# santurini/vsrlab

Measured on AMD Instinct MI355X. Metric: LR frames/sec fwd+bwd, BasicVSR 4x 540p 7-frame clip, 1->8 MI355X, higher is better.
Workload: dtype bf16; 1 GPU; BasicVSR(mid=64,res_blocks=30,x4) fwd+Charbonnier+bwd+clip+Adam, 540x960->2160x3840, 7-frame clip, 2 clips per GPU (BASELINE configs[1]); clips_per_gpu=2, frames=7, res_blocks=30, parallelism=single GPU, arena=full, train_flow=False, trunk_chains=True

## Files before the change

### vsrlab_amd/csrc/common.h

```cpp
#pragma once
#include <hip/hip_runtime.h>
#include <stdint.h>

#define VSR_OK 0
#define VSR_ERR_BADARG (-1)
#define VSR_ERR_UNSUPPORTED (-2)
#define VSR_ERR_HIP (-3)
#define VSR_ERR_WORKSPACE (-4)

#define VSR_F32 0
#define VSR_BF16 1

typedef __bf16 bf16_t;
typedef __attribute__((ext_vector_type(8))) __bf16 bf16x8_t;
typedef __attribute__((ext_vector_type(4))) __bf16 bf16x4_t;
typedef __attribute__((ext_vector_type(4))) short s16x4_t;
typedef __attribute__((ext_vector_type(16))) float f32x16_t;
typedef __attribute__((ext_vector_type(4))) float f32x4_t;

#define VSR_MAX_SRC 4
#define VSR_MAX_Z 4

enum { ACT_NONE = 0, ACT_RELU = 1, ACT_LEAKY = 2 };
enum { MASK_NONE = 0, MASK_RELU = 1, MASK_LEAKY = 2, MASK_RELU_BITS = 3, MASK_LEAKY_BITS = 4 };
enum { EPI_NHWC = 0, EPI_PLANAR = 1 };

struct ConvArgs {
    const void* src[VSR_MAX_SRC];
    long long src_nstride[VSR_MAX_SRC];
    int src_oy[VSR_MAX_SRC], src_ox[VSR_MAX_SRC];
    int in_step, Hs, Ws;
    int N, H, W;
    const void* wpack;
    long long w_zstride;
    const float* bias;
    int bias_zstride;
    int nz;
    void* dst[VSR_MAX_Z];
    long long dst_nstride;
    int out_step, Hd, Wd;
    int out_oy[VSR_MAX_Z], out_ox[VSR_MAX_Z];
    int CD;
    int cout_real;
    int act;
    const void* res[VSR_MAX_Z];
    const void* aux[VSR_MAX_Z];
    int mask_mode;
    const float* pres;
    const float* base_lr;
    long long base_nstride;
    int base_h, base_w, base_scale;
    void* sign_out[VSR_MAX_Z];
    const void* sign_bits[VSR_MAX_Z];
    float leaky_slope;
    int planar_c;
    int unshuffle;
    long long unshuffle_plane;
};
static inline __host__ __device__ float vsr_slope(float s) { return s != 0.f ? s : 0.1f; }

#define VSR_WG_MAXSEG 8
struct WgradArgs {
    const void* x[VSR_WG_MAXSEG];
    const void* dy[VSR_WG_MAXSEG];
    long long x_nstride, dy_nstride;
    int nseg;
    int N, H, W;
    int x_step, x_oy, x_ox, Hx, Wx;
    int dy_step, dy_oy, dy_ox, Hy, Wy;
    float* slab;
    int tap_begin;
    int x_ctotal, x_coff;
    int dy_ctotal, dy_coff;
    int dy_planar_c;
    int slab_stride;
    int ntiles_x, ntiles_y;
    int pair_ksplit, pair_nsl, pair_ncob, pair_views;
};

static inline __host__ __device__ int cdiv(int a, int b) { return (a + b - 1) / b; }

static inline __host__ __device__ int pm_ws(int W) { return (W + 31) >> 5; }
static inline __host__ __device__ long long pm_image_elems(int H, int W, int C) { return (long long)H * pm_ws(W) * 32 * C; }
static inline __host__ __device__ long long pm_off(int y, int x, int chunk, int W, int C) {
    const int seg = x >> 5;
    return (((long long)y * pm_ws(W) + seg) * (C >> 3) + chunk) * 256 + (x & 31) * 8;
}

static inline __host__ __device__ int pm_acc_chan(int mb, int row) { return 8 * (4 * (mb >> 1) + (row >> 2)) + 4 * (mb & 1) + (row & 3); }
#define PM_LANE_PIXEL(l15) (((l15) >= 4 && (l15) < 12) ? 2 * ((l15) - 4) : ((l15) < 4 ? 2 * (l15) + 1 : 2 * ((l15) - 8) + 1))

struct TileWalk { int first, end, stride; };
static inline __device__ TileWalk xcd_tile_walk(int total, int block, int nblocks) {
    TileWalk w;
    if (nblocks >= 8 && (nblocks & 7) == 0) {
        const int xcd = block & 7, j = block >> 3;
        const int lo = (int)((long long)xcd * total / 8), hi = (int)((long long)(xcd + 1) * total / 8);
        w.first = lo + j; w.end = hi; w.stride = nblocks >> 3;
    } else {
        w.first = block; w.end = total; w.stride = nblocks;
    }
    return w;
}

#define VSR_MAX_DEVICES 32
struct VsrDevOnce { bool done[VSR_MAX_DEVICES] = {}; };
static inline int vsr_set_max_dynamic_lds(VsrDevOnce& once, const void* kernel, int bytes) {
    int dev = 0;
    if (hipGetDevice(&dev) != hipSuccess) return VSR_ERR_HIP;
    if (dev < 0 || dev >= VSR_MAX_DEVICES) return VSR_ERR_UNSUPPORTED;
    if (!__atomic_load_n(&once.done[dev], __ATOMIC_ACQUIRE)) {
        if (hipFuncSetAttribute(kernel, hipFuncAttributeMaxDynamicSharedMemorySize, bytes) != hipSuccess) return VSR_ERR_HIP;
        __atomic_store_n(&once.done[dev], true, __ATOMIC_RELEASE);
    }
    return VSR_OK;
}

static inline int vsr_num_cus() {
    static int cus[VSR_MAX_DEVICES] = {};
    int dev = 0;
    if (hipGetDevice(&dev) != hipSuccess || dev < 0 || dev >= VSR_MAX_DEVICES) return 256;
    int v = __atomic_load_n(&cus[dev], __ATOMIC_RELAXED);
    if (v == 0) {
        hipDeviceProp_t prop;
        v = (hipGetDeviceProperties(&prop, dev) == hipSuccess && prop.multiProcessorCount > 0) ? prop.multiProcessorCount : 256;
        __atomic_store_n(&cus[dev], v, __ATOMIC_RELAXED);
    }
    return v;
}

#include <cstdlib>
struct VsrEnvSwitches {
    bool generic_conv, generic_wgrad, single_stream;
    int wide2_max_wg;
};
static inline const VsrEnvSwitches& vsr_env() {
    static const VsrEnvSwitches s = [] {
        auto on = [](const char* n) { const char* e = getenv(n); return e && e[0] == '1'; };
        VsrEnvSwitches v;
        v.generic_conv = on("VSRLAB_AMD_GENERIC_CONV");
        v.generic_wgrad = on("VSRLAB_AMD_GENERIC_WGRAD");
        v.single_stream = on("VSRLAB_AMD_SINGLE_STREAM");
        const char* e = getenv("VSRLAB_AMD_WIDE2_MAX_WG");
        v.wide2_max_wg = e ? atoi(e) : 0;
        return v;
    }();
    return s;
}

#define HIP_CHECK_RET(expr)                                   \
    do {                                                      \
        hipError_t _e = (expr);                               \
        if (_e != hipSuccess) return VSR_ERR_HIP;             \
    } while (0)
```

### vsrlab_amd/csrc/kernels.h

```cpp
#pragma once
#include "common.h"

int vsr_launch_conv(int dtype, int ks, int nsrc, int ca, int cb, int last_planar, int cout_t, int epi,
                    const ConvArgs& a, hipStream_t st);
int vsr_launch_sign_bits_c64(const void* x_pm, void* bits, int N, int H, int W, hipStream_t st);

enum { CHAIN_RELU = 0,
       CHAIN_SKIP = 1,
       CHAIN_MASK = 2 };
#define VSR_CHAIN_MAX_LAYERS 64
struct ChainLayer { unsigned src, dst, res, sbits, sout, w, bias; int variant; };
struct ChainArgs {
    char* base;
    unsigned* sync;
    int N, H, W, nlayers;
    ChainLayer layer[VSR_CHAIN_MAX_LAYERS];
};
size_t vsr_chain_sync_bytes(int nlayers, int N, int H, int W);
int vsr_launch_conv3x3_chain(const ChainArgs& a, int num_cus, hipStream_t st);
void vsr_wgrad_slab_dims(int ks, int cx, int cout, int* coutp, int* cxp, int* stride);
int vsr_launch_wgrad(int dtype, int ks, int cx, int x_planar, int cout, int dy_planar, const WgradArgs& a, int nwg,
                     int* nslabs, hipStream_t st);
int vsr_launch_wgrad_reduce(const float* slab, int nwg, int ks, int cx, int cout, int cout_real, int cin_real, float* gw,
                            int I_total, int i_off, int o_mul, int o_add, float* gb, int accumulate, hipStream_t st);
int vsr_launch_warp_fwd(int dtype, const void* in, const float* flow, void* out, int N, int H, int W, int C,
                        long long flow_nstride, hipStream_t st, int border = 0);
int vsr_launch_warp_bwd(int dtype, const void* dout, const float* flow, float* dacc, int N, int H, int W, int C,
                        long long flow_nstride, hipStream_t st, int border = 0);
int vsr_launch_warp_bwd_gather(int dtype, const void* dout, const float* flow, const void* dtop, long long* S, int* far_count, void* out,
                               int N, int H, int W, int C, long long flow_nstride, hipStream_t st);
int vsr_launch_add_cast(int dtype, const void* a, const float* s, void* out, int N, int H, int W, int C, hipStream_t st);
int vsr_launch_planar_to_pm(int dtype, const float* in, void* out, int N, int Cin, int H, int W, int C, hipStream_t st);
int vsr_launch_pm_to_planar(int dtype, const void* in, float* out, int N, int Cout, int H, int W, int C, hipStream_t st);
int vsr_launch_resize_norm(const float* in, float* out, const float* mean, const float* std, int F, int h, int w, int hu,
                           int wu, hipStream_t st);
int vsr_launch_avgpool2(const float* in, float* out, long long planes, int h, int w, hipStream_t st);
int vsr_launch_spynet_prepare(int dtype, const float* frames, const float* flow_prev, float* flow_up, void* x16, int n,
                              int t, int P, int pair_mode, int h, int w, int level0, hipStream_t st);
int vsr_launch_flow_out(const float* in, float* out, int P, int hu, int wu, int h, int w, hipStream_t st);
int vsr_launch_warp_bwd_flow(int dtype, const void* in, const void* dout, const float* flow, float* dflow, int N, int H, int W,
                             int C, long long flow_nstride, hipStream_t st, int border = 0);
int vsr_launch_spynet_dres(int dtype, const float* dflow, const float* res, void* out, int P, int h, int w, hipStream_t st);
int vsr_launch_spynet_prepare_bwd(int dtype, const void* dx16, const float* dflow_l, const float* frames, const float* flow_up,
                                  float* dflow_prev, float* dframes, int n, int t, int P, int pair_mode, int h, int w, hipStream_t st);
int vsr_launch_avgpool2_bwd_add(const float* dcoarse, float* dfine, long long planes, int h, int w, hipStream_t st);
int vsr_launch_resize_norm_bwd(const float* dnorm, float* dframes, const float* std, int F, int h, int w, int hu, int wu, hipStream_t st);
int vsr_launch_bilinear4_bwd(const float* dsr, float* dlr, long long planes, int h, int w, hipStream_t st, int scale = 4);
int vsr_launch_flow_out_bwd(const float* dout, float* din, int P, int hu, int wu, int h, int w, hipStream_t st);
int vsr_launch_add_f32(const float* a, const float* b, float* out, long long n, hipStream_t st);
int vsr_launch_c64_to_planar(const ConvArgs& a, hipStream_t st);
int vsr_launch_last2_wgrad(const void* x, const float* dy, long long dy_nstride, float* slab, int slab_stride, int N, int H, int W,
                           int* nslabs, hipStream_t st, int pc = 3);
int vsr_launch_last2_dgrad(const float* dsr, long long dsr_nstride, const float* w, const void* aux, void* dst, int N, int H, int W,
                           int mask_mode, hipStream_t st, const void* sign_bits = nullptr, float slope = 0.f);
struct VsrPackDesc {
    const float* w; void* dst;
    int total, blk0;
    short KK, RP, CPd, r_real, c_real, I_total, i_off, o_mul, o_add;
    unsigned char mode, dtype;
};
#define VSR_PACK_BATCH 80
int vsr_launch_pack_multi(const VsrPackDesc* descs, int n, hipStream_t st);
int vsr_launch_pack_weights(int dtype, const float* w, void* dst, int KK, int RP, int CPd, int r_real, int c_real,
                            int I_total, int i_off, int o_mul, int o_add, int mode, hipStream_t st);
int vsr_charbonnier_scratch_floats_impl();
int vsr_launch_charbonnier_grad(const float* sr, const float* hr, float* dsr, float* loss_acc, float* scratch, long long n, float eps,
                                hipStream_t st);

struct VsrWideConv {
    const void* x; int xC, Hx, Wx, in_step, nsl;
    int N, H, W;
    const void* wpack; const float* bias;
    void* y; int yC, Hy, Wy, out_step, ncob;
    int act; float slope;
    void* y_act; const void* res; void* y_pre; const void* aux;
    const void* wpack2;
};
// ... 15 lines not shown
```

### vsrlab_amd/csrc/recipes.h

```cpp
#pragma once
#include <vector>
#include "host.h"

inline constexpr int NSPY = 5;
inline constexpr int SPY_CI[NSPY] = {8, 32, 64, 32, 16};
inline constexpr int SPY_CO[NSPY] = {32, 64, 32, 16, 2};
inline constexpr int SPY_CIP[NSPY] = {16, 32, 64, 32, 16};
inline constexpr int SPY_COP[NSPY] = {32, 64, 32, 32, 32};
inline constexpr int SPY_CD[NSPY] = {32, 64, 32, 16, 0};
inline constexpr int SPY_DK[NSPY] = {32, 64, 32, 16, 16};
inline constexpr int SPY_DROWS[NSPY] = {32, 32, 64, 32, 32};

struct Ctx {
    char* ws;
    hipStream_t st;
    int dtype;
    int C, CO;
    size_t es;
    float* slab;
    mutable std::vector<VsrPackDesc>* batch = nullptr;
    Ctx(char* ws_, hipStream_t st_, int dtype_, int C_ = 64, float* slab_ = nullptr)
        : ws(ws_), st(st_), dtype(dtype_), C(C_), CO(C_ < 32 ? 32 : C_), es(esize(dtype_)), slab(slab_) {}
    void* at(size_t off) const { return ws + off; }
    const float* fat(size_t off) const { return reinterpret_cast<const float*>(ws + off); }
// ... 10 lines not shown
        if (unshuffle) set_unshuffle(a, N, H, W);
        const int rc = vsr_launch_conv(dtype, ks, 1, C, C, 0, CO, EPI_NHWC, a, st);
        if (rc == VSR_OK && sign_out && dtype == VSR_BF16 && vsr_env().generic_conv) return vsr_launch_sign_bits_c64(y, sign_out, N, H, W, st);
        return rc;
    }
    int conv_planar3(const void* x, const void* wpack, const float* bias, float* y, long long y_nstride, const float* pres, int N, int H, int W) const {
        ConvArgs a = conv_args(N, H, W, C);
        a.src[0] = x; a.wpack = wpack; a.bias = bias; a.cout_real = 3; a.dst[0] = y; a.dst_nstride = y_nstride; a.pres = pres;
        return vsr_launch_conv(dtype, 3, 1, C, C, 0, 32, EPI_PLANAR, a, st);
    }

    int pack_ps(const float* w, void* dst, int mode) const {
        for (int z = 0; z < 4; ++z) CK(pack(w, (char*)dst + (size_t)z * 9 * CO * C * es, 9, CO, C, C, C, C, 0, 4, z, mode));
        return VSR_OK;
    }
    int pack_ps_bias(const float* b, float* dst) const {
        for (int z = 0; z < 4; ++z) CK(pack_bias(b, dst + z * C, C, 4, z));
        return VSR_OK;
    }
    int conv_ps(const void* x, const void* wpack, const float* bias4, void* y, int N, int H, int W, int act = ACT_NONE, float slope = 0.f) const {
        ConvArgs a = conv_args(N, H, W, C);
        a.src[0] = x; a.wpack = wpack; a.w_zstride = 9 * CO * C; a.bias = bias4; a.bias_zstride = C; a.nz = 4; a.act = act; a.leaky_slope = slope;
        a.out_step = 2; a.Hd = 2 * H; a.Wd = 2 * W; a.dst_nstride = pm_image_elems(2 * H, 2 * W, C);
        for (int z = 0; z < 4; ++z) { a.dst[z] = y; a.out_oy[z] = z >> 1; a.out_ox[z] = z & 1; }
        return vsr_launch_conv(dtype, 3, 1, C, C, 0, CO, EPI_NHWC, a, st);
    }
    int conv_ps_dgrad(const void* dy, const void* wpackd, void* dx, const void* aux, int mask, int N, int H, int W, const void* sign_bits = nullptr,
                      bool dy_planes = false, bool dx_planes = false) const {
        if (dtype == VSR_BF16 && C == 64) {
            for (int z = 0; z < 4; ++z) {
                ConvArgs a = conv_args(N, H, W, C);
                if (dy_planes) {
                    a.src[0] = (const char*)dy + (size_t)z * plane_elems(N, 2 * H, 2 * W) * es;
                } else {
                    a.in_step = 2; a.Hs = 2 * H; a.Ws = 2 * W;
                    a.src[0] = dy; a.src_oy[0] = z >> 1; a.src_ox[0] = z & 1; a.src_nstride[0] = pm_image_elems(2 * H, 2 * W, C);
                }
                a.wpack = (const char*)wpackd + (size_t)z * 9 * C * C * es; a.dst[0] = dx;
                a.res[0] = z > 0 ? dx : nullptr;
                if (dx_planes) set_unshuffle(a, N, H, W);
                if (z == 3) { a.aux[0] = aux; a.mask_mode = mask; a.sign_bits[0] = aux ? sign_bits : nullptr; }
                int rc = vsr_launch_conv(dtype, 3, 1, 64, 64, 0, 64, EPI_NHWC, a, st);
                if (rc != VSR_OK) return rc;
            }
            return VSR_OK;
        }
        ConvArgs a = conv_args(N, H, W, C);
        a.nz = 1; a.in_step = 2; a.Hs = 2 * H; a.Ws = 2 * W;
        for (int s = 0; s < 4; ++s) { a.src[s] = dy; a.src_oy[s] = s >> 1; a.src_ox[s] = s & 1; a.src_nstride[s] = pm_image_elems(2 * H, 2 * W, C); }
        a.wpack = wpackd; a.dst[0] = dx; a.aux[0] = aux; a.mask_mode = mask;
        return vsr_launch_conv(dtype, 3, 4, C, C, 0, CO, EPI_NHWC, a, st);
    }
    int ps_wgrads(const void* const* x, const void* const* dy, int nseg, bool dy_planes, int N, int H, int W, float* gw, float* gb, int accumulate) const {
        for (int z = 0; z < 4; ++z) {
            WgradArgs a = wg_base(N, H, W, C, C);
            a.nseg = nseg;
            for (int i = 0; i < nseg; ++i) {
                a.x[i] = x[i];
                a.dy[i] = dy_planes ? (const char*)dy[i] + (size_t)z * plane_elems(N, 2 * H, 2 * W) * es : dy[i];
            }
            if (!dy_planes) { a.dy_step = 2; a.dy_oy = z >> 1; a.dy_ox = z & 1; a.Hy = 2 * H; a.Wy = 2 * W; a.dy_nstride = pm_image_elems(2 * H, 2 * W, C); }
            CK(wgrad(a, {3, C, false, C, false}, {C, C, gw, C, 0, 4, z, gb, accumulate}));
        }
        return VSR_OK;
    }

    int pack_stem(const float* w, void* dst, bool cat) const {
        const int I_total = cat ? C + 3 : 3;
        if (cat) CK(pack(w, dst, 9, CO, C, C, C, I_total, 3, 1, 0, 0));
        return pack(w, (char*)dst + (cat ? (size_t)9 * CO * C * es : 0), 9, CO, 16, C, 3, I_total, 0, 1, 0, 0);
    }
    int pack_stem_dgrad(const float* w, void* dst) const { return pack(w, dst, 9, CO, C, C, C, C + 3, 3, 1, 0, 1); }
    int pack_stem_dlr(const float* w, void* dst, bool cat) const { return pack(w, dst, 9, 32, C, 3, C, cat ? C + 3 : 3, 0, 1, 0, 1); }
    int stem(bool cat, const void* feat, const float* lr, long long lr_nstride, const void* wpack, const float* bias, void* y, int act, float slope,
             int N, int H, int W) const {
        ConvArgs a = conv_args(N, H, W, C);
        a.wpack = wpack; a.bias = bias; a.dst[0] = y; a.act = act; a.leaky_slope = slope;
        a.src[cat ? 1 : 0] = lr; a.src_nstride[cat ? 1 : 0] = lr_nstride;
        if (!cat) return vsr_launch_conv(dtype, 3, 1, 16, 16, 1, CO, EPI_NHWC, a, st);
        a.src[0] = feat;
        return vsr_launch_conv(dtype, 3, 2, C, 16, 1, CO, EPI_NHWC, a, st);
    }
    int stem_wgrads(bool cat, WgradArgs& a_lr, WgradArgs& a_feat, float* gw, float* gb, int accumulate) const {
        const int I_total = cat ? C + 3 : 3;
        CK(wgrad(a_lr, {3, 16, true, C, false}, {C, 3, gw, I_total, 0, 1, 0, gb, accumulate}));
        if (cat && a_feat.nseg) CK(wgrad_cc(3, a_feat, gw, I_total, 3, nullptr, accumulate));
        return VSR_OK;
    }

    int pack_spy(int j, const float* w, void* dst, int mode) const {
        if (mode == 0) return pack(w, dst, 49, SPY_COP[j], SPY_CIP[j], SPY_CO[j], SPY_CI[j], SPY_CI[j], 0, 1, 0, 0);
        return pack(w, dst, 49, SPY_DROWS[j], SPY_DK[j], SPY_CI[j], SPY_CO[j], SPY_CI[j], 0, 1, 0, 1);
    }
    int spy_conv(int j, const void* x, const void* wpack, const float* bias, void* y, int act, float slope, const float* pres, int N, int H, int W) const {
        ConvArgs a = conv_args(N, H, W, SPY_CD[j]);
        a.src[0] = x; a.src_nstride[0] = pm_image_elems(H, W, SPY_CIP[j]);
        a.wpack = wpack; a.bias = bias; a.act = act; a.leaky_slope = slope; a.cout_real = SPY_CO[j]; a.dst[0] = y;
        if (j < NSPY - 1) return vsr_launch_conv(dtype, 7, 1, SPY_CIP[j], SPY_CIP[j], 0, SPY_COP[j], EPI_NHWC, a, st);
        a.dst_nstride = (long long)2 * H * W; a.pres = pres;
        return vsr_launch_conv(dtype, 7, 1, 16, 16, 0, 32, EPI_PLANAR, a, st);
    }
    int spy_dgrad(int j, const void* dy, const void* wpackd, void* dx, const void* aux, int N, int H, int W) const {
        const int CI = SPY_CIP[j], DK = SPY_DK[j];
        ConvArgs a = conv_args(N, H, W, CI);
        a.src[0] = dy; a.src_nstride[0] = pm_image_elems(H, W, DK);
        a.wpack = wpackd; a.dst[0] = dx; a.cout_real = j == 0 ? 8 : CI;
// ... 43 lines not shown
```

### vsrlab_amd/csrc/wgrad_mfma.hip

```cpp
#include <cstdlib>
#include "kernels.h"

namespace {

constexpr int TW = 32, TH = 8, NTHREADS = 256;

template <typename T> struct WElt;
template <> struct WElt<bf16_t> { static constexpr int CHB = 16; typedef uint4 chunk_t; };
struct wchunk32_t { uint4 a, b; };
template <> struct WElt<float> { static constexpr int CHB = 32; typedef wchunk32_t chunk_t; };

template <typename T> __device__ __forceinline__ typename WElt<T>::chunk_t wzero();
template <> __device__ __forceinline__ uint4 wzero<bf16_t>() { return make_uint4(0, 0, 0, 0); }
template <> __device__ __forceinline__ wchunk32_t wzero<float>() { wchunk32_t z; z.a = make_uint4(0, 0, 0, 0); z.b = z.a; return z; }

__device__ __forceinline__ uint4 wchunk3(float a, float b, float c, bf16_t*) {
    union { bf16_t h[8]; uint4 u; } t; t.u = make_uint4(0, 0, 0, 0);
    t.h[0] = (bf16_t)a; t.h[1] = (bf16_t)b; t.h[2] = (bf16_t)c; return t.u;
}
__device__ __forceinline__ wchunk32_t wchunk3(float a, float b, float c, float*) {
    wchunk32_t t; t.a = make_uint4(__float_as_uint(a), __float_as_uint(b), __float_as_uint(c), 0); t.b = make_uint4(0, 0, 0, 0); return t;
}
__device__ __forceinline__ void chunk_sum(const uint4& v, float* s) {
    union { uint4 u; bf16_t h[8]; } t; t.u = v;
// ... 186 lines not shown
#pragma unroll
                        for (int j = 0; j < 8; ++j) {
                            const int py = row * TW + xk + 2 * j + h;
                            const float av = *reinterpret_cast<const float*>(ly + lds_addr<T, CPY>(py, chy));
#pragma unroll
                            for (int i = 0; i < NTAP; ++i) {
                                const int tap = a.tap_begin + tap0 + i * TAPSPLIT;
                                if (tap0 + i * TAPSPLIT < KT) {
                                    const int ky = tap / KS, kx = tap - ky * KS;
                                    const int px = (row + ky) * TWH + xk + kx + 2 * j + h;
                                    const float bv = *reinterpret_cast<const float*>(lx + lds_addr<T, CPX>(px, chx));
                                    acc[i] = __builtin_amdgcn_mfma_f32_32x32x2f32(av, bv, acc[i], 0, 0, 0);
                                }
                            }
                        }
                    }
                }
            }
        }
    }

    float* slab = a.slab + (long long)blockIdx.x * a.slab_stride;
#pragma unroll
    for (int i = 0; i < NTAP; ++i) {
        const int tap = a.tap_begin + tap0 + i * TAPSPLIT;
        if (tap0 + i * TAPSPLIT < KT) {
#pragma unroll
            for (int r = 0; r < 16; ++r) {
                const int co = cb * 32 + (r & 3) + 8 * (r >> 2) + 4 * h;
                slab[((long long)tap * COUTP + co) * CXP + ib * 32 + l31] = acc[i][r];
            }
        }
    }
    __syncthreads();
    float* red = reinterpret_cast<float*>(smem);
#pragma unroll
    for (int j = 0; j < 8; ++j) red[tid * 8 + j] = bsum[j];
    __syncthreads();
    if (tid < COUTP) {
        float s = 0.f;
        if (DYPLANAR) {
            if (tid < 3) for (int t = 0; t < NTHREADS; ++t) s += red[t * 8 + tid];
        } else if (tid < COUT) {
            const int c = tid >> 3, j = tid & 7;
            for (int t = c; t < NTHREADS; t += CPY) s += red[t * 8 + j];
        }
        slab[(long long)KK * COUTP * CXP + tid] = s;
    }
}

__global__ void wgrad_reduce_kernel(const float* slab, int nwg, int slab_stride, int KK, int COUTP, int CXP,
                                    int cout_real, int cin_real, float* gw, int I_total, int i_off, int o_mul, int o_add,
                                    float* gb, int accumulate) {
    __shared__ float part[4][64];
    const int total = KK * cout_real * cin_real;
    const int e = threadIdx.x & 63, grp = threadIdx.x >> 6;
    const int idx = blockIdx.x * 64 + e;
    const float* p = nullptr;
    float* d = nullptr;
    if (idx < total) {
        const int ci = idx % cin_real;
        const int co = (idx / cin_real) % cout_real;
        const int tap = idx / (cin_real * cout_real);
        p = slab + ((long long)tap * COUTP + co) * CXP + ci;
        d = gw + ((long long)(co * o_mul + o_add) * I_total + i_off + ci) * KK + tap;
    } else if (gb && idx < total + cout_real) {
        const int co = idx - total;
        p = slab + (long long)KK * COUTP * CXP + co;
        d = gb + co * o_mul + o_add;
    }
    float s = 0.f;
    if (p) {
        int w = grp;
        for (; w + 44 < nwg; w += 48) {
            float v[12];
#pragma unroll
            for (int k = 0; k < 12; ++k) v[k] = p[(long long)(w + 4 * k) * slab_stride];
            s += (v[0] + v[1]) + (v[2] + v[3]);
            s += (v[4] + v[5]) + (v[6] + v[7]);
            s += (v[8] + v[9]) + (v[10] + v[11]);
        }
        for (; w + 12 < nwg; w += 16) {
            const float v0 = p[(long long)w * slab_stride], v1 = p[(long long)(w + 4) * slab_stride];
            const float v2 = p[(long long)(w + 8) * slab_stride], v3 = p[(long long)(w + 12) * slab_stride];
            s += (v0 + v1) + (v2 + v3);
        }
        for (; w < nwg; w += 4) s += p[(long long)w * slab_stride];
    }
    part[grp][e] = s;
    __syncthreads();
    if (grp == 0 && d) {
        s = (part[0][e] + part[1][e]) + (part[2][e] + part[3][e]);
        *d = accumulate ? *d + s : s;
    }
}

__global__ void wgrad_reduce_pairs_kernel(const float* __restrict__ slab, int slab_stride, int ksplit, int nsl, int ncob, int views,
                                          float* __restrict__ gw, int cin_total) {
    __shared__ float part[4][64];
    const int e = threadIdx.x & 63, grp = threadIdx.x >> 6;
    const int idx = blockIdx.x * 64 + e;
    const int pair = blockIdx.y;
    const int sl = pair % nsl, o = (pair / nsl) % ncob, v = pair / (nsl * ncob);
    const int ci = idx & 63, co = (idx >> 6) & 63, tap = idx >> 12;
    float* d = nullptr;
    if (views == 1) {
// ... 1 lines not shown
    } else {
        const int dy = tap / 3 - 1, dx = tap % 3 - 1;
        const int ky = (v >> 1) == 0 ? (dy >= 0 ? 2 * dy + 1 : -1) : (dy <= 0 ? 2 * (dy + 1) : -1);
        const int kx = (v & 1) == 0 ? (dx >= 0 ? 2 * dx + 1 : -1) : (dx <= 0 ? 2 * (dx + 1) : -1);
        if (ky >= 0 && kx >= 0) d = gw + ((long long)(o * 64 + co) * cin_total + sl * 64 + ci) * 16 + ky * 4 + kx;
    }
    float s = 0.f;
    if (d) {
        const float* p = slab + (long long)pair * ksplit * slab_stride + idx;
        for (int w = grp; w < ksplit; w += 4) s += p[(long long)w * slab_stride];
    }
    part[grp][e] = s;
    __syncthreads();
    if (grp == 0 && d) *d += (part[0][e] + part[1][e]) + (part[2][e] + part[3][e]);
}

template <typename T, int KS, int CX, bool XP, int COUT, bool DP>
int launch_wgrad_inst(const WgradArgs& a0, int nwg, hipStream_t st) {
    constexpr int TWH = TW + KS - 1, THH = TH + KS - 1;
    constexpr int CHB = WElt<T>::CHB;
    constexpr int LDS_T = THH * TWH * (CX / 8) * CHB + TH * TW * (COUT / 8) * CHB;
    constexpr int LDS = LDS_T > NTHREADS * 8 * 4 ? LDS_T : NTHREADS * 8 * 4;
    static_assert(LDS <= 160 * 1024, "wgrad tiles do not fit LDS");
    auto kern = wgrad_kernel<T, KS, CX, XP, COUT, DP>;
    static VsrDevOnce once;
    { const int rc = vsr_set_max_dynamic_lds(once, reinterpret_cast<const void*>(kern), LDS); if (rc != VSR_OK) return rc; }
    WgradArgs a = a0;
    a.ntiles_x = cdiv(a.W, TW);
    a.ntiles_y = cdiv(a.H, TH);
    for (int tb = 0; tb < KS * KS; tb += (KS == 7 ? 7 : KS * KS)) {
        a.tap_begin = tb;
        hipLaunchKernelGGL(kern, dim3(nwg), dim3(NTHREADS), LDS, st, a);
        HIP_CHECK_RET(hipGetLastError());
    }
    return VSR_OK;
}

__device__ uint4 g_zero_chunk[2];

constexpr int XS = 36, YS = 35;
constexpr int XROW = 8 * XS * 16, YROW = 8 * YS * 16;
constexpr int DXB = (TH + 2) * XROW;
constexpr int DYB = TH * YROW;
constexpr int DSET = DXB + DYB;
constexpr int DX_SLOTS = (TH + 2) * 8 * XS, DY_SLOTS = TH * 8 * YS;
constexpr int DX_PIECES = DX_SLOTS / 64;
constexpr int DY_PIECES = DY_SLOTS / 64;
constexpr int DNT = 512;
static_assert(DX_SLOTS % 64 == 0 && DY_SLOTS % 64 == 0, "whole DMA pieces");

#ifdef VSR_CLOCK
__device__ unsigned long long g_wclk[256 * 4];
#endif
__global__ __launch_bounds__(DNT, 2) void wgrad3x3_c64_pc_kernel(const WgradArgs a) {
    extern __shared__ __attribute__((aligned(16))) char smem[];
    const int tid = threadIdx.x, lane = tid & 63, wave = tid >> 6;
    const int role = __builtin_amdgcn_readfirstlane(wave >> 2);
    const int w4 = __builtin_amdgcn_readfirstlane(wave & 3);
#ifdef VSR_CLOCK
    unsigned long long clk_t0 = 0, clk_r0 = 0, clk_bar = 0, clk_tiles = 0;
    if (tid == 0) { clk_t0 = __builtin_amdgcn_s_memtime(); clk_r0 = __builtin_amdgcn_s_memrealtime(); }
#endif
    const int tiles_per_img = a.ntiles_x * a.ntiles_y;
    const int per_seg = a.N * tiles_per_img;
    const int total = a.nseg * per_seg;
    TileWalk walk = xcd_tile_walk(total, blockIdx.x, gridDim.x);
    int x_coff = a.x_coff, dy_coff = a.dy_coff, x_oy = a.x_oy, x_ox = a.x_ox;
    int slab_idx = blockIdx.x;
    if (a.pair_ksplit > 0) {
        const int kq = a.pair_ksplit >> 3, xcd = blockIdx.x & 7, j = blockIdx.x >> 3;
        const int pair = j / kq, part = xcd + 8 * (j - pair * kq);
        const int s = pair % a.pair_nsl, o = (pair / a.pair_nsl) % a.pair_ncob, v = pair / (a.pair_nsl * a.pair_ncob);
        x_coff = s * 8; dy_coff = o * 8;
        if (a.pair_views > 1) { x_oy = v >> 1; x_ox = v & 1; }
        walk.first = (int)((long long)total * part / a.pair_ksplit);
        walk.end = (int)((long long)total * (part + 1) / a.pair_ksplit);
        walk.stride = 1;
        slab_idx = pair * a.pair_ksplit + part;
    }
    float* slab = a.slab + (long long)slab_idx * a.slab_stride;

    if (role == 1) {
        const char* zsrc = reinterpret_cast<const char*>(g_zero_chunk);
        const int xcp = (a.x_ctotal ? a.x_ctotal : 64) >> 3, ycp = (a.dy_ctotal ? a.dy_ctotal : 64) >> 3;
        constexpr int NPIECE = (DX_PIECES + DY_PIECES) / 4;
        static_assert((DX_PIECES + DY_PIECES) % 4 == 0, "even split over 4 producer waves");
        int rel[NPIECE];
        unsigned padmask = 0;
#pragma unroll
        for (int i = 0; i < NPIECE; ++i) {
            const int piece = w4 + 4 * i;
            if (piece < DX_PIECES) {
                const int idx = piece * 64 + lane;
                const int row = idx / (8 * XS), rem = idx - row * (8 * XS);
                const int c = rem / XS, tx = rem - c * XS;
                const int dx = (tx - 1) * a.x_step + x_ox;
                rel[i] = (((((row - 1) * a.x_step) * pm_ws(a.Wx) + (dx >> 5)) * xcp + c) * 256 + (dx & 31) * 8) * 2;
                if (tx >= TW + 2) padmask |= 1u << i;
            } else {
                const int idx = (piece - DX_PIECES) * 64 + lane;
                const int row = idx / (8 * YS), rem = idx - row * (8 * YS);
                const int c = rem / YS, tx = rem - c * YS - (c & 1);
                const int dx = (tx < 0 ? 0 : tx) * a.dy_step + a.dy_ox;
                rel[i] = ((((row * a.dy_step) * pm_ws(a.Wy) + (dx >> 5)) * ycp + c) * 256 + (dx & 31) * 8) * 2;
                if (tx < 0 || tx >= TW) padmask |= 1u << i;
            }
        }
        struct { int T, seg, n, ty, tx, sseg, sn, sty, stx; } it;
        {
            int r = walk.first;
            it.T = r; it.seg = r / per_seg; r -= it.seg * per_seg; it.n = r / tiles_per_img; r -= it.n * tiles_per_img;
            it.ty = r / a.ntiles_x; it.tx = r - it.ty * a.ntiles_x;
            r = walk.stride;
            it.sseg = r / per_seg; r -= it.sseg * per_seg; it.sn = r / tiles_per_img; r -= it.sn * tiles_per_img;
            it.sty = r / a.ntiles_x; it.stx = r - it.sty * a.ntiles_x;
        }
        auto advance = [&]() {
            it.T += walk.stride;
            it.tx += it.stx; if (it.tx >= a.ntiles_x) { it.tx -= a.ntiles_x; ++it.ty; }
            it.ty += it.sty; if (it.ty >= a.ntiles_y) { it.ty -= a.ntiles_y; ++it.n; }
            it.n += it.sn; if (it.n >= a.N) { it.n -= a.N; ++it.seg; }
            it.seg += it.sseg;
        };
        int cseg = -1;
        const char *xseg = nullptr, *yseg = nullptr;
        auto issue = [&](int s) {
            if (it.seg != cseg) {
                cseg = it.seg;
                xseg = reinterpret_cast<const char*>(a.x[cseg]);
                yseg = reinterpret_cast<const char*>(a.dy[cseg]);
            }
            const int ty0 = it.ty * TH, tx0 = it.tx * TW;
            const char* xb = xseg + (long long)it.n * a.x_nstride * 2;
            const char* yb = yseg + (long long)it.n * a.dy_nstride * 2;
            const char* xo = xb + pm_off(ty0 * a.x_step + x_oy, tx0 * a.x_step, x_coff, a.Wx, xcp * 8) * 2;
            const char* yo = yb + pm_off(ty0 * a.dy_step + a.dy_oy, tx0 * a.dy_step, dy_coff, a.Wy, ycp * 8) * 2;
            char* lxs = smem + s * DSET;
            const bool interior = ty0 >= 1 && ty0 + TH < a.H && tx0 >= 1 && tx0 + TW < a.W;
#pragma unroll
            for (int i = 0; i < NPIECE; ++i) {
                const int piece = w4 + 4 * i;
                const bool isx = piece < DX_PIECES;
                const char* src = (isx ? xo : yo) + rel[i];
                const bool pad = (padmask >> i) & 1u;
                bool valid = true;
                if (!interior && !pad) {
                    if (isx) {
                        const int idx = piece * 64 + lane;
                        const int row = idx / (8 * XS), tx = (idx - row * (8 * XS)) % XS;
                        const int vy = ty0 + row - 1, vx = tx0 + tx - 1;
                        valid = vy >= 0 && vy < a.H && vx >= 0 && vx < a.W;
                    } else {
                        const int idx = (piece - DX_PIECES) * 64 + lane;
                        const int row = idx / (8 * YS), rem = idx - row * (8 * YS), c = rem / YS, tx = rem - c * YS - (c & 1);
                        valid = ty0 + row < a.H && tx0 + tx < a.W;
                    }
                }
                if (!valid) src = zsrc;
                char* dst = isx ? lxs + piece * 1024 : lxs + DXB + (piece - DX_PIECES) * 1024;
                if (!pad) __builtin_amdgcn_global_load_lds((const __attribute__((address_space(1))) void*)src,
                                                           (__attribute__((address_space(3))) void*)dst, 16, 0, 0);
            }
        };
        float bsum[8];
#pragma unroll
        for (int j = 0; j < 8; ++j) bsum[j] = 0.f;
        const int pt = tid - 256;
        int cur = 0;
        if (it.T < walk.end) issue(0);
        asm volatile("s_waitcnt vmcnt(0)" ::: "memory");
        __syncthreads();
        while (it.T < walk.end) {
            const unsigned lyb = (unsigned)(cur * DSET + DXB + (pt & 7) * (YS * 16) + ((pt >> 3) + (pt & 1)) * 16);
            advance();
            if (it.T < walk.end) issue(cur ^ 1);
            uint4 bq[8];
            asm volatile("ds_read_b128 %0, %8\n\tds_read_b128 %1, %8 offset:%9\n\tds_read_b128 %2, %8 offset:%10\n\tds_read_b128 %3, %8 offset:%11\n\t"
                         "ds_read_b128 %4, %8 offset:%12\n\tds_read_b128 %5, %8 offset:%13\n\tds_read_b128 %6, %8 offset:%14\n\tds_read_b128 %7, %8 offset:%15\n\t"
                         "s_waitcnt lgkmcnt(0)"
                         : "=&v"(bq[0]), "=&v"(bq[1]), "=&v"(bq[2]), "=&v"(bq[3]), "=&v"(bq[4]), "=&v"(bq[5]), "=&v"(bq[6]), "=&v"(bq[7])
                         : "v"(lyb), "i"(YROW), "i"(2 * YROW), "i"(3 * YROW), "i"(4 * YROW), "i"(5 * YROW), "i"(6 * YROW), "i"(7 * YROW) : "memory");
#pragma unroll
            for (int i = 0; i < 8; ++i) chunk_sum(bq[i], bsum);
            asm volatile("s_waitcnt vmcnt(0)" ::: "memory");
            __syncthreads();
            cur ^= 1;
        }
        __syncthreads();
        float* red = reinterpret_cast<float*>(smem);
// ... 49 lines not shown
            PC_TOP PC_GRP(5, 2, 0, 3) PC_GRP(5, 1, 6, 3) PC_GRP(5, 0, 12, 3)
            PC_TOP PC_GRP(6, 2, 0, 3) PC_GRP(6, 1, 6, 3) PC_GRP(6, 0, 12, 3)
            PC_TOP PC_GRP(7, 2, 0, 3) PC_GRP(7, 1, 6, 3) PC_GRP(7, 0, 12, 3)
            PC_TOP PC_GRP(8, 2, 0, 2) PC_GRP(8, 1, 6, 2)
            PC_TOP PC_GRP(9, 2, 0, 1)
#undef PC_TOP
#undef PC_GRP
#undef PC_PAIR
#undef PC_LDB
#undef PC_LDA
#undef PC_TRR
#ifdef VSR_CLOCK
            unsigned long long b0; asm volatile("s_waitcnt lgkmcnt(0)\n\ts_memtime %0\n\ts_waitcnt lgkmcnt(0)" : "=s"(b0) :: "memory");
#endif
            __syncthreads();
#ifdef VSR_CLOCK
            unsigned long long b1; asm volatile("s_memtime %0\n\ts_waitcnt lgkmcnt(0)" : "=s"(b1) :: "memory");
            clk_bar += b1 - b0; ++clk_tiles;
#endif
            cur ^= 1;
        }
#pragma unroll
        for (int t = 0; t < 9; ++t)
#pragma unroll
            for (int m = 0; m < 2; ++m)
#pragma unroll
                for (int n = 0; n < 2; ++n)
#pragma unroll
                    for (int j = 0; j < 4; ++j)
                        slab[((long long)t * 64 + cb * 32 + m * 16 + 4 * q + j) * 64 + ib * 32 + n * 16 + l15] = acc[t][m][n][j];
        __syncthreads();
        __syncthreads();
        if (tid < 64) {
            const float* red = reinterpret_cast<const float*>(smem);
            float s = 0.f;
            const int c = tid >> 3, j = tid & 7;
            for (int t = c; t < 256; t += 8) s += red[t * 8 + j];
            slab[9 * 64 * 64 + tid] = s;
        }
    }
#ifdef VSR_CLOCK
    if (tid == 0 && blockIdx.x < 256) {
        g_wclk[blockIdx.x * 4 + 0] = __builtin_amdgcn_s_memtime() - clk_t0;
        g_wclk[blockIdx.x * 4 + 1] = __builtin_amdgcn_s_memrealtime() - clk_r0;
        g_wclk[blockIdx.x * 4 + 2] = clk_bar;
        g_wclk[blockIdx.x * 4 + 3] = clk_tiles;
    }
#endif
}

int launch_wgrad_pc(const WgradArgs& a0, int nwg, hipStream_t st) {
    constexpr int LDS = 2 * DSET;
    static VsrDevOnce once;
    { const int rc = vsr_set_max_dynamic_lds(once, reinterpret_cast<const void*>(wgrad3x3_c64_pc_kernel), LDS); if (rc != VSR_OK) return rc; }
    WgradArgs a = a0;
    a.ntiles_x = cdiv(a.W, TW);
    a.ntiles_y = cdiv(a.H, TH);
    hipLaunchKernelGGL(wgrad3x3_c64_pc_kernel, dim3(nwg), dim3(DNT), LDS, st, a);
    HIP_CHECK_RET(hipGetLastError());
    return VSR_OK;
}

}

#ifdef VSR_CLOCK
extern "C" int vsr_debug_read_wclk(unsigned long long* host_out) {
    return hipMemcpyFromSymbol(host_out, HIP_SYMBOL(g_wclk), sizeof(unsigned long long) * 256 * 4) == hipSuccess ? 0 : -3;
}
#endif



#define VSR_WGRAD_SHAPES(X)           \
    X(3, 64, false, 64, false)         \
    X(3, 16, true, 64, false)          \
    X(3, 64, false, 16, true)          \
    X(1, 64, false, 64, false)         \
    X(7, 16, false, 32, false)         \
    X(7, 32, false, 64, false)         \
    X(7, 64, false, 32, false)         \
    X(7, 32, false, 32, false)        \
    X(7, 32, false, 16, false)         \
    X(7, 16, false, 16, false)         \
     \
    X(3, 16, false, 16, false)         \
    X(3, 32, false, 32, false)         \
    X(3, 16, true, 16, false)          \
    X(3, 16, true, 32, false)          \
    X(1, 16, false, 16, false)         \
    X(1, 32, false, 32, false)        \
    X(3, 16, false, 64, false)         \
    X(3, 32, false, 64, false)        \
    X(3, 16, false, 16, true)          \
    X(3, 32, false, 16, true)

int vsr_launch_wgrad7x7_pc(int cx, int cout, const WgradArgs& a, int max_slabs, int* nslabs, hipStream_t st);

void vsr_wgrad_slab_dims(int ks, int cx, int cout, int* coutp, int* cxp, int* stride) {
    const int ncb = cout >= 32 ? cout / 32 : 1, nib = cx >= 32 ? cx / 32 : 1;
    *coutp = ncb * 32;
    *cxp = nib * 32;
    *stride = ks * ks * (*coutp) * (*cxp) + (*coutp);
}

int vsr_launch_wgrad(int dtype, int ks, int cx, int x_planar, int cout, int dy_planar,
                     const WgradArgs& a, int nwg, int* nslabs, hipStream_t st) {
    if (a.nseg < 1 || a.nseg > VSR_WG_MAXSEG || nwg < 1 || !nslabs) return VSR_ERR_BADARG;
    *nslabs = nwg;
    {
        const bool force_generic = vsr_env().generic_wgrad;
        if (!force_generic && dtype == VSR_BF16 && ks == 3 && cx == 64 && !x_planar && cout == 64 && !dy_planar && nwg >= 2) {
            *nslabs = nwg / 2;
            return launch_wgrad_pc(a, nwg / 2, st);
        }
    }
    if (!vsr_env().generic_wgrad && dtype == VSR_BF16 && ks == 3 && cx == 64 && !x_planar && cout == 16 && dy_planar && a.nseg == 1 && a.x_step == 1 &&
        a.dy_step == 1 && !a.x_oy && !a.x_ox && !a.dy_oy && !a.dy_ox && a.Hx == a.H && a.Wx == a.W && a.Hy == a.H && a.Wy == a.W && !a.x_ctotal && !a.x_coff &&
        a.x_nstride == pm_image_elems(a.H, a.W, 64)) {
        const int rc = vsr_launch_last2_wgrad(a.x[0], reinterpret_cast<const float*>(a.dy[0]), a.dy_nstride, a.slab, a.slab_stride, a.N, a.H, a.W, nslabs, st,
                                              a.dy_planar_c ? a.dy_planar_c : 3);
        if (rc != VSR_ERR_UNSUPPORTED) return rc;
        *nslabs = nwg;
    }
    if (!vsr_env().generic_wgrad && dtype == VSR_BF16 && ks == 7 && !x_planar && !dy_planar) {
        const int rc = vsr_launch_wgrad7x7_pc(cx, cout, a, nwg, nslabs, st);
        if (rc != VSR_ERR_UNSUPPORTED) return rc;
        *nslabs = nwg;
    }
#define X(KS, CX, XP, COUT, DP)                                                                        \
    if (ks == KS && cx == CX && (x_planar != 0) == XP && cout == COUT && (dy_planar != 0) == DP) {    \
        if (dtype == VSR_BF16) return launch_wgrad_inst<bf16_t, KS, CX, XP, COUT, DP>(a, nwg, st);    \
        if (dtype == VSR_F32) {                                                                       \
            if constexpr (KS == 7 && CX == 64) return VSR_ERR_UNSUPPORTED;                             \
            else return launch_wgrad_inst<float, KS, CX, XP, COUT, DP>(a, nwg, st);                   \
        }                                                                                             \
        return VSR_ERR_BADARG;                                                                        \
    }
    VSR_WGRAD_SHAPES(X)
#undef X
    return VSR_ERR_UNSUPPORTED;
}

int vsr_launch_wgrad_reduce(const float* slab, int nwg, int ks, int cx, int cout, int cout_real, int cin_real,
                            float* gw, int I_total, int i_off, int o_mul, int o_add, float* gb, int accumulate,
                            hipStream_t st) {
    int coutp, cxp, stride;
    vsr_wgrad_slab_dims(ks, cx, cout, &coutp, &cxp, &stride);
    const int total = ks * ks * cout_real * cin_real + (gb ? cout_real : 0);
    hipLaunchKernelGGL(wgrad_reduce_kernel, dim3(cdiv(total, 64)), dim3(256), 0, st, slab, nwg, stride, ks * ks,
                       coutp, cxp, cout_real, cin_real, gw, I_total, i_off, o_mul, o_add, gb, accumulate);
    HIP_CHECK_RET(hipGetLastError());
    return VSR_OK;
}

int vsr_launch_wgrad_pairs(int dtype, const WgradArgs& a0, int nsl, int ncob, int views, int ksplit, float* gw, int cin_total, hipStream_t st) {
    if (dtype != VSR_BF16) return VSR_ERR_UNSUPPORTED;
    if (nsl < 1 || ncob < 1 || (views != 1 && views != 4) || ksplit < 8 || (ksplit & 7) || a0.nseg < 1 || a0.nseg > VSR_WG_MAXSEG) return VSR_ERR_BADARG;
    const int npairs = nsl * ncob * views;
    if ((long long)npairs * ksplit > VSR_WGRAD_MAX_PAIR_SLABS) return VSR_ERR_BADARG;
    constexpr int LDS = 2 * DSET;
    static VsrDevOnce once;
    { const int rc = vsr_set_max_dynamic_lds(once, reinterpret_cast<const void*>(wgrad3x3_c64_pc_kernel), LDS); if (rc != VSR_OK) return rc; }
    WgradArgs a = a0;
    a.ntiles_x = cdiv(a.W, TW);
    a.ntiles_y = cdiv(a.H, TH);
    a.pair_ksplit = ksplit; a.pair_nsl = nsl; a.pair_ncob = ncob; a.pair_views = views;
    hipLaunchKernelGGL(wgrad3x3_c64_pc_kernel, dim3(npairs * ksplit), dim3(DNT), LDS, st, a);
    HIP_CHECK_RET(hipGetLastError());
    hipLaunchKernelGGL(wgrad_reduce_pairs_kernel, dim3(9 * 64, npairs), dim3(256), 0, st, a.slab, a.slab_stride, ksplit, nsl, ncob, views, gw, cin_total);
    HIP_CHECK_RET(hipGetLastError());
    return VSR_OK;
}
```

Before: 59.68 LR frames/s.

## Batch four pixel-shuffle phase wgrads into one launch with z-indexed reduce

Replaces the per-phase loop of four separate weight-gradient launches plus reductions for the pixel-shuffle upsampling conv with a single templated kernel launch whose blocks are split across the four phases, and a single reduce launch using a second grid dimension over phases. Blocks are mapped so that phase members share XCD locality for tile reuse. The aim is to cut launch overhead and tail underutilisation from four small grids. In exchange, each phase now gets a fixed number of groups (up to 64), which may change parallelism per phase, and the slab must hold four times the slices.

```diff
diff --git a/vsrlab_amd/csrc/common.h b/vsrlab_amd/csrc/common.h
--- a/vsrlab_amd/csrc/common.h
+++ b/vsrlab_amd/csrc/common.h
@@ -76,6 +76,8 @@
     int slab_stride;
     int ntiles_x, ntiles_y;
     int pair_ksplit, pair_nsl, pair_ncob, pair_views;
+    int ps_nz, ps_dy_view;
+    long long ps_dy_zstride;
 };
 
 static inline __host__ __device__ int cdiv(int a, int b) { return (a + b - 1) / b; }
@@ -91,7 +93,7 @@
 #define PM_LANE_PIXEL(l15) (((l15) >= 4 && (l15) < 12) ? 2 * ((l15) - 4) : ((l15) < 4 ? 2 * (l15) + 1 : 2 * ((l15) - 8) + 1))
 
 struct TileWalk { int first, end, stride; };
-static inline __device__ TileWalk xcd_tile_walk(int total, int block, int nblocks) {
+static inline __host__ __device__ TileWalk xcd_tile_walk(int total, int block, int nblocks) {
     TileWalk w;
     if (nblocks >= 8 && (nblocks & 7) == 0) {
         const int xcd = block & 7, j = block >> 3;
@@ -101,6 +103,14 @@
         w.first = block; w.end = total; w.stride = nblocks;
     }
     return w;
+}
+static inline __host__ __device__ void ps_phase_member(int block, int groups, int& group, int& z) {
+    if (groups >= 8 && (groups & 7) == 0) {
+        const int xcd = block & 7, j = block >> 3;
+        z = j & 3; group = xcd + 8 * (j >> 2);
+    } else {
+        z = block & 3; group = block >> 2;
+    }
 }
 
 #define VSR_MAX_DEVICES 32
diff --git a/vsrlab_amd/csrc/kernels.h b/vsrlab_amd/csrc/kernels.h
--- a/vsrlab_amd/csrc/kernels.h
+++ b/vsrlab_amd/csrc/kernels.h
@@ -22,7 +22,9 @@
 int vsr_launch_wgrad(int dtype, int ks, int cx, int x_planar, int cout, int dy_planar, const WgradArgs& a, int nwg,
                      int* nslabs, hipStream_t st);
 int vsr_launch_wgrad_reduce(const float* slab, int nwg, int ks, int cx, int cout, int cout_real, int cin_real, float* gw,
-                            int I_total, int i_off, int o_mul, int o_add, float* gb, int accumulate, hipStream_t st);
+                            int I_total, int i_off, int o_mul, int o_add, float* gb, int accumulate, hipStream_t st, int nz = 1);
+#define VSR_WGRAD_PS_GROUPS 64
+int vsr_launch_wgrad_ps(const WgradArgs& a, int* groups, hipStream_t st);
 int vsr_launch_warp_fwd(int dtype, const void* in, const float* flow, void* out, int N, int H, int W, int C,
                         long long flow_nstride, hipStream_t st, int border = 0);
 int vsr_launch_warp_bwd(int dtype, const void* dout, const float* flow, float* dacc, int N, int H, int W, int C,
diff --git a/vsrlab_amd/csrc/recipes.h b/vsrlab_amd/csrc/recipes.h
--- a/vsrlab_amd/csrc/recipes.h
+++ b/vsrlab_amd/csrc/recipes.h
@@ -86,6 +86,19 @@
         return vsr_launch_conv(dtype, 3, 4, C, C, 0, CO, EPI_NHWC, a, st);
     }
     int ps_wgrads(const void* const* x, const void* const* dy, int nseg, bool dy_planes, int N, int H, int W, float* gw, float* gb, int accumulate) const {
+        if (dtype == VSR_BF16 && C == 64 && !vsr_env().generic_wgrad) {
+            if (!gw && !gb) return VSR_OK;
+            if (!gw) return VSR_ERR_BADARG;
+            WgradArgs a = wg_base(N, H, W, C, C);
+            a.nseg = nseg; a.ps_nz = 4;
+            for (int i = 0; i < nseg; ++i) { a.x[i] = x[i]; a.dy[i] = dy[i]; }
+            if (dy_planes) a.ps_dy_zstride = plane_elems(N, 2 * H, 2 * W);
+            else { a.ps_dy_view = 1; a.dy_step = 2; a.Hy = 2 * H; a.Wy = 2 * W; a.dy_nstride = pm_image_elems(2 * H, 2 * W, C); }
+            a.slab = slab; a.slab_stride = wgrad_slab_stride3();
+            int groups = 0;
+            CK(vsr_launch_wgrad_ps(a, &groups, st));
+            return vsr_launch_wgrad_reduce(slab, groups, 3, C, C, C, C, gw, C, 0, 4, 0, gb, accumulate, st, 4);
+        }
         for (int z = 0; z < 4; ++z) {
             WgradArgs a = wg_base(N, H, W, C, C);
             a.nseg = nseg;
diff --git a/vsrlab_amd/csrc/wgrad_mfma.hip b/vsrlab_amd/csrc/wgrad_mfma.hip
--- a/vsrlab_amd/csrc/wgrad_mfma.hip
+++ b/vsrlab_amd/csrc/wgrad_mfma.hip
@@ -262,6 +262,8 @@
 __global__ void wgrad_reduce_kernel(const float* slab, int nwg, int slab_stride, int KK, int COUTP, int CXP,
                                     int cout_real, int cin_real, float* gw, int I_total, int i_off, int o_mul, int o_add,
                                     float* gb, int accumulate) {
+    slab += (long long)blockIdx.y * nwg * slab_stride;
+    o_add += blockIdx.y;
     __shared__ float part[4][64];
     const int total = KK * cout_real * cin_real;
     const int e = threadIdx.x & 63, grp = threadIdx.x >> 6;
@@ -369,6 +371,7 @@
 #ifdef VSR_CLOCK
 __device__ unsigned long long g_wclk[256 * 4];
 #endif
+template <bool PS>
 __global__ __launch_bounds__(DNT, 2) void wgrad3x3_c64_pc_kernel(const WgradArgs a) {
     extern __shared__ __attribute__((aligned(16))) char smem[];
     const int tid = threadIdx.x, lane = tid & 63, wave = tid >> 6;
@@ -384,7 +387,17 @@
     TileWalk walk = xcd_tile_walk(total, blockIdx.x, gridDim.x);
     int x_coff = a.x_coff, dy_coff = a.dy_coff, x_oy = a.x_oy, x_ox = a.x_ox;
     int slab_idx = blockIdx.x;
-    if (a.pair_ksplit > 0) {
+    int ps_oy = 0, ps_ox = 0;
+    long long ps_zbytes = 0;
+    if constexpr (PS) {
+        const int groups = gridDim.x >> 2;
+        int group, z;
+        ps_phase_member(blockIdx.x, groups, group, z);
+        walk = xcd_tile_walk(total, group, groups);
+        slab_idx = z * groups + group;
+        if (a.ps_dy_view) { ps_oy = z >> 1; ps_ox = z & 1; }
+        ps_zbytes = (long long)z * a.ps_dy_zstride * 2;
+    } else if (a.pair_ksplit > 0) {
         const int kq = a.pair_ksplit >> 3, xcd = blockIdx.x & 7, j = blockIdx.x >> 3;
         const int pair = j / kq, part = xcd + 8 * (j - pair * kq);
         const int s = pair % a.pair_nsl, o = (pair / a.pair_nsl) % a.pair_ncob, v = pair / (a.pair_nsl * a.pair_ncob);
@@ -418,7 +431,7 @@
                 const int idx = (piece - DX_PIECES) * 64 + lane;
                 const int row = idx / (8 * YS), rem = idx - row * (8 * YS);
                 const int c = rem / YS, tx = rem - c * YS - (c & 1);
-                const int dx = (tx < 0 ? 0 : tx) * a.dy_step + a.dy_ox;
+                const int dx = (tx < 0 ? 0 : tx) * a.dy_step + a.dy_ox + (PS ? ps_ox : 0);
                 rel[i] = ((((row * a.dy_step) * pm_ws(a.Wy) + (dx >> 5)) * ycp + c) * 256 + (dx & 31) * 8) * 2;
                 if (tx < 0 || tx >= TW) padmask |= 1u << i;
             }
@@ -445,13 +458,13 @@
             if (it.seg != cseg) {
                 cseg = it.seg;
                 xseg = reinterpret_cast<const char*>(a.x[cseg]);
-                yseg = reinterpret_cast<const char*>(a.dy[cseg]);
+                yseg = reinterpret_cast<const char*>(a.dy[cseg]) + (PS ? ps_zbytes : 0);
             }
             const int ty0 = it.ty * TH, tx0 = it.tx * TW;
             const char* xb = xseg + (long long)it.n * a.x_nstride * 2;
             const char* yb = yseg + (long long)it.n * a.dy_nstride * 2;
             const char* xo = xb + pm_off(ty0 * a.x_step + x_oy, tx0 * a.x_step, x_coff, a.Wx, xcp * 8) * 2;
-            const char* yo = yb + pm_off(ty0 * a.dy_step + a.dy_oy, tx0 * a.dy_step, dy_coff, a.Wy, ycp * 8) * 2;
+            const char* yo = yb + pm_off(ty0 * a.dy_step + a.dy_oy + (PS ? ps_oy : 0), tx0 * a.dy_step, dy_coff, a.Wy, ycp * 8) * 2;
             char* lxs = smem + s * DSET;
             const bool interior = ty0 >= 1 && ty0 + TH < a.H && tx0 >= 1 && tx0 + TW < a.W;
 #pragma unroll
@@ -607,11 +620,23 @@
 int launch_wgrad_pc(const WgradArgs& a0, int nwg, hipStream_t st) {
     constexpr int LDS = 2 * DSET;
     static VsrDevOnce once;
-    { const int rc = vsr_set_max_dynamic_lds(once, reinterpret_cast<const void*>(wgrad3x3_c64_pc_kernel), LDS); if (rc != VSR_OK) return rc; }
+    { const int rc = vsr_set_max_dynamic_lds(once, reinterpret_cast<const void*>(wgrad3x3_c64_pc_kernel<false>), LDS); if (rc != VSR_OK) return rc; }
     WgradArgs a = a0;
     a.ntiles_x = cdiv(a.W, TW);
     a.ntiles_y = cdiv(a.H, TH);
-    hipLaunchKernelGGL(wgrad3x3_c64_pc_kernel, dim3(nwg), dim3(DNT), LDS, st, a);
+    hipLaunchKernelGGL(wgrad3x3_c64_pc_kernel<false>, dim3(nwg), dim3(DNT), LDS, st, a);
+    HIP_CHECK_RET(hipGetLastError());
+    return VSR_OK;
+}
+
+int launch_wgrad_pc_ps(const WgradArgs& a0, int groups, hipStream_t st) {
+    constexpr int LDS = 2 * DSET;
+    static VsrDevOnce once;
+    { const int rc = vsr_set_max_dynamic_lds(once, reinterpret_cast<const void*>(wgrad3x3_c64_pc_kernel<true>), LDS); if (rc != VSR_OK) return rc; }
+    WgradArgs a = a0;
+    a.ntiles_x = cdiv(a.W, TW);
+    a.ntiles_y = cdiv(a.H, TH);
+    hipLaunchKernelGGL(wgrad3x3_c64_pc_kernel<true>, dim3(4 * groups), dim3(DNT), LDS, st, a);
     HIP_CHECK_RET(hipGetLastError());
     return VSR_OK;
 }
@@ -698,14 +723,29 @@
 
 int vsr_launch_wgrad_reduce(const float* slab, int nwg, int ks, int cx, int cout, int cout_real, int cin_real,
                             float* gw, int I_total, int i_off, int o_mul, int o_add, float* gb, int accumulate,
-                            hipStream_t st) {
+                            hipStream_t st, int nz) {
+    if (nz < 1) return VSR_ERR_BADARG;
     int coutp, cxp, stride;
     vsr_wgrad_slab_dims(ks, cx, cout, &coutp, &cxp, &stride);
     const int total = ks * ks * cout_real * cin_real + (gb ? cout_real : 0);
-    hipLaunchKernelGGL(wgrad_reduce_kernel, dim3(cdiv(total, 64)), dim3(256), 0, st, slab, nwg, stride, ks * ks,
+    hipLaunchKernelGGL(wgrad_reduce_kernel, dim3(cdiv(total, 64), nz), dim3(256), 0, st, slab, nwg, stride, ks * ks,
                        coutp, cxp, cout_real, cin_real, gw, I_total, i_off, o_mul, o_add, gb, accumulate);
     HIP_CHECK_RET(hipGetLastError());
     return VSR_OK;
+}
+
+int vsr_launch_wgrad_ps(const WgradArgs& a, int* groups, hipStream_t st) {
+    if (a.nseg < 1 || a.nseg > VSR_WG_MAXSEG || a.ps_nz != 4 || !groups || !a.slab) return VSR_ERR_BADARG;
+    const long long tiles = (long long)a.nseg * a.N * cdiv(a.H, TH) * cdiv(a.W, TW);
+    *groups = tiles < VSR_WGRAD_PS_GROUPS ? (int)tiles : VSR_WGRAD_PS_GROUPS;
+    return launch_wgrad_pc_ps(a, *groups, st);
+}
+
+extern "C" void vsr_debug_ps_wgrad_member(int block, int groups, int total_tiles, int* out) {
+    int group, z;
+    ps_phase_member(block, groups, group, z);
+    const TileWalk w = xcd_tile_walk(total_tiles, group, groups);
+    out[0] = group; out[1] = z; out[2] = w.first; out[3] = w.end; out[4] = w.stride;
 }
 
 int vsr_launch_wgrad_pairs(int dtype, const WgradArgs& a0, int nsl, int ncob, int views, int ksplit, float* gw, int cin_total, hipStream_t st) {
@@ -715,12 +755,12 @@
     if ((long long)npairs * ksplit > VSR_WGRAD_MAX_PAIR_SLABS) return VSR_ERR_BADARG;
     constexpr int LDS = 2 * DSET;
     static VsrDevOnce once;
-    { const int rc = vsr_set_max_dynamic_lds(once, reinterpret_cast<const void*>(wgrad3x3_c64_pc_kernel), LDS); if (rc != VSR_OK) return rc; }
+    { const int rc = vsr_set_max_dynamic_lds(once, reinterpret_cast<const void*>(wgrad3x3_c64_pc_kernel<false>), LDS); if (rc != VSR_OK) return rc; }
     WgradArgs a = a0;
     a.ntiles_x = cdiv(a.W, TW);
     a.ntiles_y = cdiv(a.H, TH);
     a.pair_ksplit = ksplit; a.pair_nsl = nsl; a.pair_ncob = ncob; a.pair_views = views;
-    hipLaunchKernelGGL(wgrad3x3_c64_pc_kernel, dim3(npairs * ksplit), dim3(DNT), LDS, st, a);
+    hipLaunchKernelGGL(wgrad3x3_c64_pc_kernel<false>, dim3(npairs * ksplit), dim3(DNT), LDS, st, a);
     HIP_CHECK_RET(hipGetLastError());
     hipLaunchKernelGGL(wgrad_reduce_pairs_kernel, dim3(9 * 64, npairs), dim3(256), 0, st, a.slab, a.slab_stride, ksplit, nsl, ncob, views, gw, cin_total);
     HIP_CHECK_RET(hipGetLastError());
```

Result: no change. 59.85 LR frames/s (median of 6 runs) (+0.3%).
